# WeChatCV/WeDetect

Measured on AMD Instinct MI355X. Metric: images/s at 640x640 (WeDetect-Base image tower + 80-class similarity + top-k/NMS), higher is better.
Workload: dtype f32-equivalent: fp32 operands carried as fp16 hi+lo pairs, 3 fp16-MFMA passes per product, fp32 accumulate (fp16x3); similarity GEMM, dwconv, LN, post-process native f32

## Files before the change

### wedetect_amd/csrc/split_gemm.hip

```cpp
#include <stdlib.h>
#include "split_gemm_impl.h"

namespace {

__global__ void split_weights_kernel(const float* __restrict__ w, int n, int k, int k16, float scale,
                                     unsigned short* __restrict__ out, int n_out) {
  const long long idx = (long long)blockIdx.x * blockDim.x + threadIdx.x;
  if (idx >= (long long)n_out * k16) return;
  const int row = (int)(idx / k16), kk = (int)(idx % k16);
  const float x = (kk < k && row < n) ? w[(size_t)row * k + kk] * scale : 0.0f;
  const _Float16 hi = (_Float16)x;
  const _Float16 lo = (_Float16)(x - (float)hi);
  unsigned short* o = out + (size_t)row * 2 * k16 + (kk >> 3) * 16 + (kk & 7);
  o[0] = __builtin_bit_cast(unsigned short, hi);
  o[8] = __builtin_bit_cast(unsigned short, lo);
}

template <int ACT, bool SPECIAL>
__global__ void __launch_bounds__(256) splitk_reduce_kernel(const WdConvGemm p, const float* __restrict__ ws, int splits,
                                                            float unscale, int vec_c, int vec_res, int vec_bias) {
  const long long idx = (long long)blockIdx.x * blockDim.x + threadIdx.x;
  const int nq = p.n >> 2;
  if (idx >= (long long)p.m * nq) return;
  const int m = (int)(idx / nq), n = (int)(idx - (long long)m * nq) * 4;
  const size_t plane = (size_t)p.m * p.n;
  f32x4 v = *reinterpret_cast<const f32x4*>(ws + (size_t)m * p.n + n);
  for (int s = 1; s < splits; ++s) v += *reinterpret_cast<const f32x4*>(ws + s * plane + (size_t)m * p.n + n);
  const EpiVec ev{vec_c, vec_res, vec_bias, unscale};
  epi_quad<ACT, SPECIAL>(p, epi_row<SPECIAL>(p, m), ev, m, n, v);
}

template <bool SPECIAL>
int launch_reduce(const WdConvGemm& p, const float* ws, int splits, float unscale, hipStream_t st) {
  const long long total = (long long)p.m * (p.n >> 2);
  const dim3 grid((unsigned)((total + 255) / 256)), block(256);
  const int vec_c = (p.ldc % 4 == 0) && wd_aligned16(p.c) && (p.out_mode == WD_OUT_ROWS || (p.n % 16 == 0));
  const int vec_res = p.res ? ((p.ldres % 4 == 0) && wd_aligned16(p.res)) : 0;
  const int vec_bias = p.bias ? wd_aligned16(p.bias) : 0;
  switch (p.act) {
    case WD_ACT_RELU: hipLaunchKernelGGL((splitk_reduce_kernel<WD_ACT_RELU, SPECIAL>), grid, block, 0, st, p, ws, splits, unscale, vec_c, vec_res, vec_bias); break;
    case WD_ACT_SILU: hipLaunchKernelGGL((splitk_reduce_kernel<WD_ACT_SILU, SPECIAL>), grid, block, 0, st, p, ws, splits, unscale, vec_c, vec_res, vec_bias); break;
    case WD_ACT_GELU: hipLaunchKernelGGL((splitk_reduce_kernel<WD_ACT_GELU, SPECIAL>), grid, block, 0, st, p, ws, splits, unscale, vec_c, vec_res, vec_bias); break;
    default: hipLaunchKernelGGL((splitk_reduce_kernel<WD_ACT_NONE, SPECIAL>), grid, block, 0, st, p, ws, splits, unscale, vec_c, vec_res, vec_bias); break;
  }
  return wd_launch_status();
}

}

extern "C" int64_t wd_split_weights_bytes(int32_t n, int32_t k) {
  if (n <= 0 || k <= 0) return 0;
  return (int64_t)((n + 7) & ~7) * ((k + 15) / 16 * 16) * 4;
}

static int split_weights_launch(const float* w, int32_t n, int32_t k, float scale, void* out, void* stream, int n_out) {
  if (!w || !out || n <= 0 || k <= 0 || !(scale > 0.0f) || !wd_aligned16(out)) return WD_ERR_BAD_ARG;
  const int k16 = (k + 15) / 16 * 16;
  const long long total = (long long)n_out * k16;
  hipLaunchKernelGGL(split_weights_kernel, dim3((unsigned)((total + 255) / 256)), dim3(256), 0,
                     static_cast<hipStream_t>(stream), w, n, k, k16, scale, static_cast<unsigned short*>(out), n_out);
  return wd_launch_status();
}

extern "C" int wd_split_weights(const float* w, int32_t n, int32_t k, float scale, void* out, void* stream) {
  return split_weights_launch(w, n, k, scale, out, stream, n);
}

extern "C" int wd_split_weights_padded(const float* w, int32_t n, int32_t k, float scale, void* out, void* stream) {
  return split_weights_launch(w, n, k, scale, out, stream, (n + 7) & ~7);
}

static int pick_split_cfg(const WdConvGemm& p) {
  const int m = p.m, n = p.n;
  const long long pad128 = (long long)((n + 127) / 128) * 128, pad64 = (long long)((n + 63) / 64) * 64;
  if (pad64 < pad128) return m >= 65536 ? 52 : 53;
  const bool plain = p.kh == 1 && p.kw == 1 && p.stride == 1 && p.pad == 0;
  if (plain && p.k >= 1024) return 55;
  const long long tiles = (long long)((m + 127) / 128) * ((n + 127) / 128);
  return tiles < 1024 ? 50 : 51;
}

long long wd_p8_workspace_floats();
bool wd_p8_persist_ok(int m, int n);
bool wd_conv_pp_ok(const WdConvGemm& p, int flags);
int wd_launch_conv_pp(const WdConvGemm& p, const void* w, float unscale, int flags, hipStream_t st, int ksplits, float* ws,
                      long long ws_floats, int variant, const float* unscale_dev = nullptr);
bool wd_conv3_ok(const WdConvGemm& p, int flags);
const char* wd_conv3_config_name(int m, int n);
int wd_launch_conv3(const WdConvGemm& p, const void* w, float unscale, int flags, hipStream_t st, int variant, int ksplits, float* ws,
                    long long ws_floats);

extern "C" int64_t wd_p8_workspace_bytes(void) { return 4 * wd_p8_workspace_floats(); }

static int pick_presplit_cfg(int m, int n, int k, bool park) {
  if (k % 32 == 0 && k >= 256 && m % 8 == 0 && n % 256 == 0) {
    const long long tiles = (long long)((m + 255) / 256) * (n / 256);
    static const int mink = [] { const char* e = getenv("WD_P8_PERSIST_MINK"); return e ? atoi(e) : 1024; }();
    if (park && k >= mink && wd_p8_persist_ok(m, n)) return 65;
    if (tiles >= 128) return 64;
  }
  if (k % 16 == 0 && n % 256 == 0 && m % 16 == 0 && m >= 131072) return 66;
  return m >= 131072 ? 63 : 60;
}

extern "C" const char* wd_conv_gemm_split_config(int32_t m, int32_t n, int32_t k, int32_t is_conv) {
  if (is_conv == 4) {
    const bool narrow = (n % 128) != 0 && ((n + 63) / 64) * 64 < ((n + 127) / 128) * 128;
    return narrow ? "fp16x3 256x64x16/8w/dma" : "fp16x3 256x128x16/8w/dma";
  }
  if (is_conv == 5) return wd_conv3_config_name(m, n);
  if ((is_conv == 2 || is_conv == 3) && k % 16 == 0) {
    switch (pick_presplit_cfg(m, n, k, is_conv == 3)) {
      case 65: return "fp16x3 256x256x32/8w/p8s";
      case 64: return "fp16x3 256x256x32/8w/p8";
      case 66: return "fp16x3 128x256x16/4w/p4";
      case 63: return "fp16x3 256x128x16/8w/pingpong";
      default: return "fp16x3 128x128x16/4w/glds";
    }
  }
  WdConvGemm q{};
  q.m = m; q.n = n; q.k = k; q.kh = q.kw = q.stride = 1;
  if (is_conv) q.kh = q.kw = 3;
  switch (pick_split_cfg(q)) {
    case 50: return "fp16x3 128x128x32/4w";
    case 51: return "fp16x3 128x128x16/4w";
    case 52: return "fp16x3 256x64x16/4w";
    case 55: return "fp16x3 128x128x32/4w/pf2";
    default: return "fp16x3 128x64x16/2w";
  }
}

static int pick_ksplits(const WdConvGemm& p, int cfg, int flags, long long ws_floats) {
  if (ws_floats <= 0 || (flags & WD_SPLIT_C) || (p.n & 3) || cfg == 55 || cfg == 63 || cfg >= 64) return 1;
  const int bm = 128, bn = (cfg == 52 || cfg == 53) ? 64 : 128, bk = (cfg == 50) ? 32 : 16;
  const long long tiles = (long long)((p.m + (cfg == 52 ? 255 : bm - 1)) / (cfg == 52 ? 256 : bm)) * ((p.n + bn - 1) / bn);
  const int nk = (p.k + bk - 1) / bk;
  if (tiles >= 128 || nk < 16) return 1;
  int s = (int)(512 / tiles);
  if (s > nk / 8) s = nk / 8;
  if (s > 16) s = 16;
  while (s > 1 && (long long)s * p.m * p.n > ws_floats) --s;
  return s < 2 ? 1 : s;
}

static int conv_gemm_split_impl(const WdConvGemm* pp, const void* w_split, float w_unscale, int32_t flags, int32_t cfg,
                                float* ws, int64_t ws_bytes, int32_t force_splits, hipStream_t st) {
  if (!pp) return WD_ERR_BAD_ARG;
  const WdConvGemm& p = *pp;
  const int rc = check_split_args(p, w_split, w_unscale);
  if (rc != WD_OK) return rc;
  if (flags & ~(WD_SPLIT_A | WD_SPLIT_C)) return WD_ERR_BAD_ARG;
  if (ws && !wd_aligned16(ws)) return WD_ERR_BAD_ARG;
  if (p.c2 && !(flags & WD_SPLIT_C)) return WD_ERR_BAD_ARG;
  const bool production = cfg < 0;
  if (cfg < 0) cfg = pick_split_cfg(p);
  const bool plain = p.kh == 1 && p.kw == 1 && p.stride == 1 && p.pad == 0;
  const bool special = p.out_mode != WD_OUT_ROWS || p.c_batch_stride > 0 || p.seg_rows > 0 || p.sigmoid ||
                       p.out_scale != 1.0f || p.out_bias != 0.0f;
  if (p.ln_stats || p.ln_u) {
    if (!p.ln_stats || !p.ln_u || flags != (WD_SPLIT_A | WD_SPLIT_C) || !plain || special || p.res || p.c2 || force_splits > 1 ||
        !wd_aligned16(p.ln_u) || (reinterpret_cast<uintptr_t>(p.ln_stats) & 7u))
      return WD_ERR_BAD_ARG;
    if (cfg == 70 || cfg == 73 || cfg == 74 || (cfg >= 75 && cfg <= 79) || (cfg >= 700 && cfg < 716)) return WD_ERR_UNSUPPORTED;
  }
  if (flags & WD_SPLIT_A) {
    const bool covered = plain && !special && !p.c2 && !((flags & WD_SPLIT_C) && p.res);
    const bool forced = cfg == 70 || cfg == 73 || cfg == 74 || (cfg >= 700 && cfg < 716);
    static const bool conv3_on = [] { const char* e = getenv("WEDETECT_CONV3"); return !(e && e[0] == '0'); }();
    if ((cfg >= 75 && cfg <= 79) || (production && conv3_on && !(force_splits == 0 && ws != nullptr))) {
      if (wd_conv3_ok(p, flags) && wd_conv_pp_ok(p, flags))
        return wd_launch_conv3(p, w_split, w_unscale, flags, st, cfg == 76 ? 2 : cfg == 77 ? 7 : cfg == 78 ? 8 : cfg == 79 ? 9 : 0, force_splits > 1 ? force_splits : 1, ws, ws ? ws_bytes / 4 : 0);
      if (cfg >= 75 && cfg <= 79) return WD_ERR_UNSUPPORTED;
    }
    if (forced || (production && !covered)) {
      if (!wd_conv_pp_ok(p, flags)) return forced || !covered ? WD_ERR_UNSUPPORTED : WD_ERR_BAD_ARG;
      const long long wsf = ws ? ws_bytes / 4 : 0;
      int splits = force_splits > 0 ? force_splits : 1;
      if (force_splits == 0 && wsf > 0 && !forced) {
        const long long tiles = (long long)((p.m + 255) / 256) * ((p.n + 127) / 128);
        const int nk = p.k / 16;
        if (tiles < 128 && nk >= 32) {
          int s2 = (int)(256 / tiles);
          if (s2 > nk / 16) s2 = nk / 16;
          if (s2 > 8) s2 = 8;
          while (s2 > 1 && (long long)s2 * p.m * p.n > wsf) --s2;
          if (s2 > 1) splits = s2;
        }
      }
      return wd_launch_conv_pp(p, w_split, w_unscale, flags, st, splits, ws, wsf,
                               cfg == 73 ? 3 : cfg == 74 ? 4 : cfg >= 700 ? cfg - 600 : 0);
    }
  }
  if (flags == WD_SPLIT_C) {
    if (!plain || special || p.res || p.c2 || p.n % 8 || p.ldc % 8 || (p.bias && !wd_aligned16(p.bias)) || !wd_aligned16(p.c))
      return WD_ERR_UNSUPPORTED;
    constexpr int VC = SVAR_XCD | SVAR_PIN | SVAR_LDSEPI | SVAR_CSPLIT;
    const long long tiles = (long long)((p.m + 127) / 128) * ((p.n + 127) / 128);
    return tiles < 1024 ? launch_split<2, 2, 2, 2, 32, VC, 1>(p, w_split, w_unscale, st)
                        : launch_split<2, 2, 2, 2, 16, VC, 1>(p, w_split, w_unscale, st);
  }
  if (flags != 0) {
    if (production && plain && !special && p.k % 16 == 0)
      cfg = pick_presplit_cfg(p.m, p.n, p.k, ws != nullptr && force_splits == 0 && ws_bytes / 4 >= wd_p8_workspace_floats() &&
                                                 p.lda % 8 == 0 && !(flags & ~(WD_SPLIT_A | WD_SPLIT_C)));
    if (cfg != 50 && cfg != 51 && cfg != 55 && cfg != 60 && cfg != 63 && cfg != 64 && cfg != 65 && cfg != 66 && !(cfg >= 640 && cfg < 768)) cfg = 51;
    if ((flags & WD_SPLIT_C) && cfg == 55) cfg = 50;
  }
  const long long ws_floats = ws ? ws_bytes / 4 : 0;
  int splits = force_splits > 0 ? force_splits : pick_ksplits(p, cfg, flags, ws_floats);
  {
    const int bk = (cfg == 50) ? 32 : 16, nk = (p.k + bk - 1) / bk;
    if (splits > nk) splits = nk;
  }
  if (splits > 1) {
    if ((flags & WD_SPLIT_C) || (p.n & 3) || cfg == 55 || cfg == 63 || cfg >= 64) return WD_ERR_UNSUPPORTED;
    if ((long long)splits * p.m * p.n > ws_floats) return WD_ERR_WORKSPACE;
  }
  int lrc;
  if (flags != 0) {
    lrc = wd_launch_presplit(p, w_split, w_unscale, cfg, flags, st, splits, ws, ws_floats);
  } else {
    switch (cfg) {
      case 41: lrc = launch_split<2, 2, 2, 4, 16, SVAR_XCD | SVAR_PIN | SVAR_LDSEPI>(p, w_split, w_unscale, st, splits, ws); break;
      case 50: lrc = launch_split<2, 2, 2, 2, 32, SVAR_XCD | SVAR_PIN | SVAR_LDSEPI>(p, w_split, w_unscale, st, splits, ws); break;
      case 51: lrc = launch_split<2, 2, 2, 2, 16, SVAR_XCD | SVAR_PIN | SVAR_LDSEPI>(p, w_split, w_unscale, st, splits, ws); break;
      case 52: lrc = launch_split<2, 2, 4, 1, 16, SVAR_XCD | SVAR_PIN | SVAR_LDSEPI>(p, w_split, w_unscale, st, splits, ws); break;
      case 53: lrc = launch_split<2, 2, 2, 1, 16, SVAR_XCD | SVAR_PIN | SVAR_LDSEPI>(p, w_split, w_unscale, st, splits, ws); break;
      case 55: lrc = launch_split<2, 2, 2, 2, 32, SVAR_XCD | SVAR_PF2 | SVAR_LDSEPI>(p, w_split, w_unscale, st); break;
      default: return WD_ERR_UNSUPPORTED;
    }
  }
  if (lrc != WD_OK || splits <= 1) return lrc;
  return special ? launch_reduce<true>(p, ws, splits, w_unscale, st) : launch_reduce<false>(p, ws, splits, w_unscale, st);
}

extern "C" int wd_conv_gemm_split(const WdConvGemm* pp, const void* w_split, float w_unscale, int32_t flags,
                                  int32_t cfg, void* stream) {
  return conv_gemm_split_impl(pp, w_split, w_unscale, flags, cfg, nullptr, 0, 0, static_cast<hipStream_t>(stream));
}

extern "C" int wd_conv_gemm_split_ws(const WdConvGemm* pp, const void* w_split, float w_unscale, int32_t flags,
                                     int32_t cfg, void* workspace, int64_t workspace_bytes, int32_t splits, void* stream) {
  if (splits < 0 || workspace_bytes < 0) return WD_ERR_BAD_ARG;
  return conv_gemm_split_impl(pp, w_split, w_unscale, flags, cfg, static_cast<float*>(workspace), workspace_bytes, splits,
                              static_cast<hipStream_t>(stream));
}

extern "C" int wd_fold_similarity(const WdConvGemm* pp, const void* w_split, float w_unscale, const float* w_unscale_dev,
                                  void* stream) {
  if (!pp || !w_unscale_dev) return WD_ERR_BAD_ARG;
  const WdConvGemm& p = *pp;
  const int rc = check_split_args(p, w_split, w_unscale);
  if (rc != WD_OK) return rc;
  if (p.kh != 1 || p.kw != 1 || p.stride != 1 || p.pad != 0 || p.c_batch_stride <= 0 || p.res || p.c2 || p.ln_stats || p.ln_u ||
      p.seg_rows > 0 || p.act != WD_ACT_NONE)
// ... 5 lines not shown
```

### wedetect_amd/csrc/split_gemm_conv3.hip

```cpp
#include <stdlib.h>
#include "split_epi_oct.h"

namespace {

constexpr int C3_BM = 256, C3_AG = 17;
constexpr int C3_AROWS = C3_AG * 16, C3_ROWB = 64;

__device__ __forceinline__ void c3_dma16(unsigned lds_addr, const unsigned char* src) {
  asm volatile("s_mov_b32 m0, %0\n\tglobal_load_lds_dwordx4 %1, off" ::"s"(lds_addr), "v"(src) : "memory", "m0");
}

template <int TN, int NBUF_ = 3>
struct C3 {
  static constexpr int WROWS = 64 * TN;
  static constexpr int WG = WROWS / 16;
  static constexpr int NG = C3_AG + 3 * WG;
  static constexpr int NJ = (NG + 7) / 8;
  static constexpr int A_BYTES = C3_AROWS * C3_ROWB;
  static constexpr int STAGE = A_BYTES + 3 * WROWS * C3_ROWB + 1024;
  static constexpr int NBUF = NBUF_;
  static constexpr int LDS = NBUF * STAGE;
  static_assert(LDS <= 160 * 1024, "LDS");
  static_assert(NJ == 6 || NJ == 4, "the counted waits of the K loop");
  static_assert(LDS >= 8 * 32 * EPI_LDT * 4, "operand LDS must hold one epilogue patch per wave");
};

#define C3_BARRIER()                          \
  do {                                        \
    __builtin_amdgcn_sched_barrier(0);        \
    asm volatile("" ::: "memory");            \
    __builtin_amdgcn_s_barrier();             \
    asm volatile("" ::: "memory");            \
    __builtin_amdgcn_sched_barrier(0);        \
  } while (0)

template <int TN, bool CSPLIT, int NB = 3, bool STAG = false>
__global__ void __launch_bounds__(512, NB == 2 ? 4 : 2)
split_conv3_kernel(const WdConvGemm p, const unsigned char* __restrict__ wsp, const float* __restrict__ zero, int k16,
                   float unscale, int nbn, int ksplits, float* __restrict__ ws) {
  using T = C3<TN, NB>;
  constexpr int TM = 2, BM = C3_BM, BN = 64 * TN, ROWB = C3_ROWB, NJ = T::NJ, NBUF = T::NBUF, DIST = NBUF - 1;
  extern __shared__ __attribute__((aligned(16))) unsigned char smem_raw[];
  const int t = threadIdx.x, lane = t & 63, wave = t >> 6;
  const int group = wave >> 2, wm = (wave >> 1) & 1, wn = wave & 1;
  int tile = blockIdx.x;
  {
    const int nwg = gridDim.x, xcd = tile & 7, idx = tile >> 3;
    const int q = nwg >> 3, r = nwg & 7;
    tile = (xcd < r ? xcd * (q + 1) : r * (q + 1) + (xcd - r) * q) + idx;
  }
  const int ntiles = gridDim.x / ksplits;
  const int ks = tile / ntiles;
  tile -= ks * ntiles;
  const int bn = tile % nbn, bm = tile / nbn;
  const int m0 = bm * BM, n0 = bn * BN;
  const int nci = p.cin >> 4, nk_all = 3 * nci;
  const int per_split = (nk_all + ksplits - 1) / ksplits;
  const int s_begin = ks * per_split;
  const int nk = (s_begin + per_split < nk_all ? s_begin + per_split : nk_all) - s_begin;

  const unsigned char* base[NJ];
  unsigned vmask[NJ];
  int kind[NJ], tapoff[NJ];
  unsigned ldst[NJ];
  const unsigned char* zp = reinterpret_cast<const unsigned char*>(zero);
#pragma unroll
  for (int j = 0; j < NJ; ++j) {
    const int g = wave + 8 * j;
    const int rl = lane >> 2;
    if (g < C3_AG) {
      const int row = g * 16 + rl;
      const int logical = (lane & 3) ^ ((row >> 2) & 3);
      const int memchunk = ((logical & 1) << 1) | ((logical >> 1) & 1);
      const long long mc = (long long)m0 - 1 + row;
      const bool ok = row < BM + 2 && mc >= 0 && mc < p.m;
      const long long mm = ok ? mc : 0;
      const int ho = (int)((mm / p.wout) % p.hout);
      base[j] = reinterpret_cast<const unsigned char*>(p.a) + mm * p.lda * 4 + memchunk * 16;
      unsigned mk = 0;
#pragma unroll
      for (int kh = 0; kh < 3; ++kh) mk |= ((unsigned)(ho + kh - 1) < (unsigned)p.hin) ? (1u << kh) : 0u;
      vmask[j] = ok ? mk : 0u;
      kind[j] = 0; tapoff[j] = 0;
      ldst[j] = (unsigned)(g * 1024);
    } else if (g < T::NG) {
      const int gw = g - C3_AG, tap = gw / T::WG, r16 = gw - tap * T::WG;
      const int row = r16 * 16 + rl;
      const int logical = (lane & 3) ^ ((row >> 2) & 3);
      const int memchunk = ((logical & 1) << 1) | ((logical >> 1) & 1);
      const int n = n0 + row;
      const bool ok = n < p.n;
      base[j] = wsp + (size_t)(ok ? n : 0) * k16 * 4 + memchunk * 16;
      vmask[j] = ok ? 7u : 0u;
      kind[j] = 1; tapoff[j] = tap * p.cin * 4;
      ldst[j] = (unsigned)(T::A_BYTES + (tap * T::WROWS + r16 * 16) * ROWB);
    } else {
      base[j] = zp; vmask[j] = 0u; kind[j] = 2; tapoff[j] = 0;
      ldst[j] = (unsigned)(T::STAGE - 1024);
    }
  }
  const unsigned lds0 = (unsigned)(size_t)(__attribute__((address_space(3))) unsigned char*)smem_raw;
  int i_kh = s_begin / nci, i_ci = (s_begin - (s_begin / nci) * nci) * 16;
  auto issue_part = [&](int buf, auto j0_c, auto j1_c, auto last_c) {
    constexpr int J0 = decltype(j0_c)::value, J1 = decltype(j1_c)::value;
    const unsigned lbase = lds0 + buf * T::STAGE;
    const int a_off = ((i_kh - 1) * p.wout * p.lda + i_ci) * 4;
// ... 129 lines not shown
    for (int s = 0; s < nk; ++s) {
      const unsigned char* sp = smem_raw + bcur * T::STAGE;
      const bool more = s + 2 < nk;
      rd(sp, 0);
      C3_SBARRIER();
      mm();
      C3_SBARRIER();
      rd(sp, 1);
      if (more) issue_part(bfill, IC0{}, ICH{}, std::false_type{});
      C3_SBARRIER();
      mm();
      C3_SBARRIER();
      rd(sp, 2);
      if (more) {
        issue_part(bfill, ICH{}, ICN{}, std::true_type{});
        if constexpr (NJ == 6) asm volatile("s_waitcnt vmcnt(6)" ::: "memory");
        else asm volatile("s_waitcnt vmcnt(4)" ::: "memory");
      } else {
        asm volatile("s_waitcnt vmcnt(0)" ::: "memory");
      }
      C3_SBARRIER();
      mm();
      C3_SBARRIER();
      bcur = bcur == 2 ? 0 : bcur + 1;
      bfill = bfill == 2 ? 0 : bfill + 1;
    }
    if (group == 0) C3_SBARRIER();
    C3_SBARRIER();
  } else {
#pragma unroll
  for (int d = 0; d < DIST; ++d)
    if (d < nk) issue(d);
  asm volatile("s_waitcnt vmcnt(0)" ::: "memory");
  __syncthreads();
  int bcur = 0, bfill = DIST % NBUF;
  for (int s = 0; s < nk; ++s) {
    const unsigned char* sp = smem_raw + bcur * T::STAGE;
    if (s + DIST < nk) issue(bfill);
    __builtin_amdgcn_sched_barrier(0);
    tap(sp, 0);
    tap(sp, 1);
    tap(sp, 2);
    __builtin_amdgcn_sched_barrier(0);
    if (DIST == 2 && s + 2 <= nk - 1) {
      if constexpr (NJ == 6) asm volatile("s_waitcnt vmcnt(6)" ::: "memory");
      else asm volatile("s_waitcnt vmcnt(4)" ::: "memory");
    } else {
      asm volatile("s_waitcnt vmcnt(0)" ::: "memory");
    }
    __builtin_amdgcn_sched_barrier(0);
    __syncthreads();
    __builtin_amdgcn_sched_barrier(0);
    bcur = bcur == NBUF - 1 ? 0 : bcur + 1;
    bfill = bfill == NBUF - 1 ? 0 : bfill + 1;
  }
  __syncthreads();
  }

  const int mw = m0 + group * 128 + wm * 64, nw = n0 + wn * 32 * TN;
  float* patch = reinterpret_cast<float*>(smem_raw) + wave * 32 * EPI_LDT;
  if (ksplits > 1) {
    WdConvGemm pr = p;
    pr.bias = nullptr; pr.res = nullptr; pr.c2 = nullptr; pr.range_flag = nullptr;
    pr.c = ws + (size_t)ks * p.m * p.n; pr.ldc = p.n;
    pr.out_mode = WD_OUT_ROWS; pr.c_batch_stride = 0; pr.seg_rows = 0; pr.sigmoid = 0; pr.out_scale = 1.0f; pr.out_bias = 0.0f;
    pr.act = WD_ACT_NONE;
    EpiOctOperands<TM, TN, false> ops;
    ops.load(pr, mw, nw, lane);
    EpiOctWalk<0, TM, TN, WD_ACT_NONE, false, false, false>::run(pr, 1.0f, mw, nw, lane, acc, patch, ops);
    return;
  }
  epi_oct_all<TM, TN, CSPLIT, TN == 1>(p, unscale, mw, nw, lane, acc, patch);
#ifdef C3_TRACE
  if constexpr (STAG) {
    asm volatile("s_waitcnt vmcnt(0)" ::: "memory");
    if (tile == 0 && ks == 0 && (wave & 3) == 0 && ws && lane == 0) {
      unsigned long long* trc = reinterpret_cast<unsigned long long*>(ws) + (wave >> 2) * 4096;
      trc[4095] = __builtin_readcyclecounter();
    }
  }
#endif
}

template <int TN, bool CSPLIT>
__global__ void __launch_bounds__(768, 1)
split_conv3w_kernel(const WdConvGemm p, const unsigned char* __restrict__ wsp, const float* __restrict__ zero, int k16,
                    float unscale, int nbn, int ksplits, float* __restrict__ ws) {
  using T = C3<TN, 3>;
  constexpr int TM = 2, BM = C3_BM, BN = 64 * TN, ROWB = C3_ROWB;
  constexpr int NJP = (T::NG + 3) / 4;
  static_assert(4 * NJP * 1024 <= T::STAGE + 3 * 1024, "spare slots");
  static_assert(NJP == 11 || NJP == 8, "the counted waits of the producer loop");
  extern __shared__ __attribute__((aligned(16))) unsigned char smem_raw[];
  const int t = threadIdx.x, lane = t & 63;
  const int wave = __builtin_amdgcn_readfirstlane(t >> 6);
  int tile = blockIdx.x;
  {
    const int nwg = gridDim.x, xcd = tile & 7, idx = tile >> 3;
    const int q = nwg >> 3, r = nwg & 7;
    tile = (xcd < r ? xcd * (q + 1) : r * (q + 1) + (xcd - r) * q) + idx;
  }
  const int ntiles = gridDim.x / ksplits;
  const int ks = tile / ntiles;
  tile -= ks * ntiles;
  const int bn = tile % nbn, bm = tile / nbn;
  const int m0 = bm * BM, n0 = bn * BN;
  const int nci = p.cin >> 4, nk_all = 3 * nci;
  const int per_split = (nk_all + ksplits - 1) / ksplits;
  const int s_begin = ks * per_split;
  const int nk = (s_begin + per_split < nk_all ? s_begin + per_split : nk_all) - s_begin;
  const unsigned lds0 = (unsigned)(size_t)(__attribute__((address_space(3))) unsigned char*)smem_raw;
#ifdef C3_TRACE
  unsigned long long* trc = (tile == 0 && ks == 0 && (wave & 3) == 0 && ws) ? reinterpret_cast<unsigned long long*>(ws) + (wave >> 2) * 4096 : nullptr;
  int trc_i = 0;
  C3_STAMP();
#endif

  if (wave >= 8) {
    const int pw = wave - 8;
    const unsigned char* zp = reinterpret_cast<const unsigned char*>(zero);
    const unsigned char* base[NJP];
    unsigned vmask[NJP];
#pragma unroll
    for (int j = 0; j < NJP; ++j) {
      const int g = pw + 4 * j;
      const int rl = lane >> 2;
      if (g < C3_AG) {
        const int row = g * 16 + rl;
        const int logical = (lane & 3) ^ ((row >> 2) & 3);
        const int memchunk = ((logical & 1) << 1) | ((logical >> 1) & 1);
        const int mc = m0 - 1 + row;
        const bool ok = row < BM + 2 && mc >= 0 && mc < p.m;
        const unsigned mm = ok ? (unsigned)mc : 0u;
        const int ho = (int)((mm / (unsigned)p.wout) % (unsigned)p.hout);
        base[j] = reinterpret_cast<const unsigned char*>(p.a) + (size_t)mm * p.lda * 4 + memchunk * 16;
        unsigned mk = 0;
#pragma unroll
        for (int kh = 0; kh < 3; ++kh) mk |= ((unsigned)(ho + kh - 1) < (unsigned)p.hin) ? (1u << kh) : 0u;
        vmask[j] = ok ? mk : 0u;
      } else if (g < T::NG) {
        const int gw = g - C3_AG, tap = gw / T::WG, r16 = gw - tap * T::WG;
        const int row = r16 * 16 + rl;
        const int logical = (lane & 3) ^ ((row >> 2) & 3);
        const int memchunk = ((logical & 1) << 1) | ((logical >> 1) & 1);
        const int n = n0 + row;
        const bool ok = n < p.n;
        base[j] = wsp + (size_t)(ok ? n : 0) * k16 * 4 + memchunk * 16 + (size_t)tap * p.cin * 4;
        vmask[j] = ok ? 7u : 0u;
      } else {
        base[j] = zp; vmask[j] = 0u;
      }
    }
    int i_kh = s_begin / nci, i_ci = (s_begin - (s_begin / nci) * nci) * 16;
    auto issue = [&](int buf) {
      const unsigned lbase = lds0 + buf * T::STAGE;
      const int a_off = ((i_kh - 1) * p.wout * p.lda + i_ci) * 4;
      const int w_off = (i_kh * 3 * p.cin + i_ci) * 4;
#pragma unroll
      for (int j = 0; j < NJP; ++j) {
        const int g = pw + 4 * j;
        const bool is_a = g < C3_AG;
        const unsigned ldst = is_a ? (unsigned)(g * 1024)
                                   : (g < T::NG ? (unsigned)(T::A_BYTES + (((g - C3_AG) / T::WG) * T::WROWS + ((g - C3_AG) % T::WG) * 16) * ROWB)
                                                : (unsigned)(T::STAGE - 1024));
        const unsigned bit = is_a ? (vmask[j] >> i_kh) & 1u : vmask[j] & 1u;
        c3_dma16(__builtin_amdgcn_readfirstlane(lbase + ldst), bit ? base[j] + (is_a ? a_off : w_off) : zp);
      }
      i_ci += 16;
      if (i_ci == p.cin) { i_ci = 0; ++i_kh; }
    };
    if (0 < nk) issue(0);
    if (1 < nk) issue(1);
    int bfill = 2;
    for (int k = 0; k < nk; ++k) {
      if (k + 1 < nk) {
        if constexpr (NJP == 11) asm volatile("s_waitcnt vmcnt(11)" ::: "memory");
        else asm volatile("s_waitcnt vmcnt(8)" ::: "memory");
      } else {
        asm volatile("s_waitcnt vmcnt(0)" ::: "memory");
      }
      C3_SBARRIER();
      if (k + 2 < nk) issue(bfill);
      bfill = bfill == 2 ? 0 : bfill + 1;
    }
    C3_SBARRIER();
    return;
  }

  const int group = wave >> 2, wm = (wave >> 1) & 1, wn = wave & 1;
  f32x16 acc[TM][TN];
#pragma unroll
  for (int i = 0; i < TM; ++i)
#pragma unroll
    for (int j = 0; j < TN; ++j)
#pragma unroll
      for (int r = 0; r < 16; ++r) acc[i][j][r] = 0.0f;
  unsigned aoff_h[3][TM], aoff_l[3][TM], boff_h[TN], boff_l[TN];
  const int hsel = lane >> 5;
#pragma unroll
  for (int i = 0; i < TM; ++i) {
    const int q = group * 128 + wm * 64 + i * 32 + (lane & 31);
#pragma unroll
    for (int kw = 0; kw < 3; ++kw) {
      const int row = q + kw, f = (row >> 2) & 3;
      aoff_h[kw][i] = lds0 + row * ROWB + ((hsel ^ f) << 4);
      aoff_l[kw][i] = lds0 + row * ROWB + (((2 + hsel) ^ f) << 4);
    }
    const unsigned wo = (unsigned)(m0 + q) % (unsigned)p.wout;
    constexpr unsigned ZROW = (C3_BM + 8) * ROWB;
    if (wo == 0u) { aoff_h[0][i] = lds0 + ZROW; aoff_l[0][i] = lds0 + ZROW + 32; }
    if (wo == (unsigned)p.wout - 1u) { aoff_h[2][i] = lds0 + ZROW; aoff_l[2][i] = lds0 + ZROW + 32; }
  }
#pragma unroll
  for (int j = 0; j < TN; ++j) {
    const int row = wn * 32 * TN + j * 32 + (lane & 31), f = (row >> 2) & 3;
    boff_h[j] = lds0 + T::A_BYTES + row * ROWB + ((hsel ^ f) << 4);
    boff_l[j] = lds0 + T::A_BYTES + row * ROWB + (((2 + hsel) ^ f) << 4);
  }
  h8 xh[2][TM] = {}, xl[2][TM] = {}, wh[2][TN] = {}, wl[2][TN] = {};
  using K0 = std::integral_constant<int, 0>;
  using K1 = std::integral_constant<int, 1>;
  using K2 = std::integral_constant<int, 2>;
  auto tap = [&](unsigned nb, auto kwn_c, auto cur_c) {
    constexpr int KWN = decltype(kwn_c)::value, C = decltype(cur_c)::value, N = 1 - C;
    constexpr int NR = 2 * TM + 2 * TN;
    unsigned ra[NR];
#pragma unroll
    for (int i = 0; i < TM; ++i) { ra[2 * i] = nb + aoff_h[KWN][i]; ra[2 * i + 1] = nb + aoff_l[KWN][i]; }
#pragma unroll
    for (int jj = 0; jj < TN; ++jj) {
      ra[2 * TM + 2 * jj] = nb + KWN * (T::WROWS * ROWB) + boff_h[jj];
      ra[2 * TM + 2 * jj + 1] = nb + KWN * (T::WROWS * ROWB) + boff_l[jj];
    }
    asm volatile("s_waitcnt lgkmcnt(0)" ::: "memory");
    __builtin_amdgcn_s_setprio(1);
#pragma unroll
    for (int m = 0; m < 3 * TM * TN; ++m) {
      const int pass = m / (TM * TN), i = (m % (TM * TN)) / TN, jj = m % TN;
      if (pass == 0) asm volatile("v_mfma_f32_32x32x16_f16 %0, %1, %2, %0" : "+v"(acc[i][jj]) : "v"(wl[C][jj]), "v"(xh[C][i]));
      else if (pass == 1) asm volatile("v_mfma_f32_32x32x16_f16 %0, %1, %2, %0" : "+v"(acc[i][jj]) : "v"(wh[C][jj]), "v"(xl[C][i]));
      else asm volatile("v_mfma_f32_32x32x16_f16 %0, %1, %2, %0" : "+v"(acc[i][jj]) : "v"(wh[C][jj]), "v"(xh[C][i]));
      if (m < NR) {
        const int r = m;
        if (r < 2 * TM) {
          if (r & 1) asm volatile("ds_read_b128 %0, %1" : "=v"(xl[N][r >> 1]) : "v"(ra[r]) : "memory");
          else asm volatile("ds_read_b128 %0, %1" : "=v"(xh[N][r >> 1]) : "v"(ra[r]) : "memory");
        } else {
          if (r & 1) asm volatile("ds_read_b128 %0, %1" : "=v"(wl[N][(r - 2 * TM) >> 1]) : "v"(ra[r]) : "memory");
          else asm volatile("ds_read_b128 %0, %1" : "=v"(wh[N][(r - 2 * TM) >> 1]) : "v"(ra[r]) : "memory");
        }
      }
    }
    __builtin_amdgcn_s_setprio(0);
  };
  auto stage = [&](unsigned sb, unsigned sbn, auto p0_c) {
    constexpr int P0 = decltype(p0_c)::value;
    using S0 = std::integral_constant<int, P0>;
    using S1 = std::integral_constant<int, 1 - P0>;
    tap(sb, K1{}, S0{});
    tap(sb, K2{}, S1{});
    asm volatile("s_waitcnt lgkmcnt(0)" ::: "memory");
    C3_SBARRIER();
    tap(sbn, K0{}, S0{});
  };
  C3_SBARRIER();
#pragma unroll
  for (int i = 0; i < TM; ++i) {
    asm volatile("ds_read_b128 %0, %1" : "=v"(xh[0][i]) : "v"(aoff_h[0][i]) : "memory");
    asm volatile("ds_read_b128 %0, %1" : "=v"(xl[0][i]) : "v"(aoff_l[0][i]) : "memory");
  }
#pragma unroll
  for (int jj = 0; jj < TN; ++jj) {
    asm volatile("ds_read_b128 %0, %1" : "=v"(wh[0][jj]) : "v"(boff_h[jj]) : "memory");
    asm volatile("ds_read_b128 %0, %1" : "=v"(wl[0][jj]) : "v"(boff_l[jj]) : "memory");
  }
  int bcur = 0;
  for (int s = 0; s < nk; s += 2) {
    const int b1 = bcur == 2 ? 0 : bcur + 1, b2 = b1 == 2 ? 0 : b1 + 1;
    stage((unsigned)(bcur * T::STAGE), (unsigned)(b1 * T::STAGE), K0{});
    if (s + 1 < nk) stage((unsigned)(b1 * T::STAGE), (unsigned)(b2 * T::STAGE), K1{});
    bcur = b2;
  }
  asm volatile("s_waitcnt lgkmcnt(0)" ::: "memory");

  const int mw = m0 + group * 128 + wm * 64, nw = n0 + wn * 32 * TN;
  float* patch = reinterpret_cast<float*>(smem_raw) + wave * 32 * EPI_LDT;
  if (ksplits > 1) {
    WdConvGemm pr = p;
    pr.bias = nullptr; pr.res = nullptr; pr.c2 = nullptr; pr.range_flag = nullptr;
    pr.c = ws + (size_t)ks * p.m * p.n; pr.ldc = p.n;
    pr.out_mode = WD_OUT_ROWS; pr.c_batch_stride = 0; pr.seg_rows = 0; pr.sigmoid = 0; pr.out_scale = 1.0f; pr.out_bias = 0.0f;
    pr.act = WD_ACT_NONE;
    EpiOctOperands<TM, TN, false> ops;
    ops.load(pr, mw, nw, lane);
    EpiOctWalk<0, TM, TN, WD_ACT_NONE, false, false, false>::run(pr, 1.0f, mw, nw, lane, acc, patch, ops);
    return;
  }
  epi_oct_all<TM, TN, CSPLIT, TN == 1>(p, unscale, mw, nw, lane, acc, patch);
#ifdef C3_TRACE
  asm volatile("s_waitcnt vmcnt(0)" ::: "memory");
  if (trc && lane == 0) trc[4095] = __builtin_readcyclecounter();
#endif
}

template <int TN, bool CSPLIT>
int launch_conv3w(const WdConvGemm& p, const void* wsp, float unscale, hipStream_t st, int ksplits = 1, float* ws = nullptr) {
  using T = C3<TN, 3>;
  constexpr int BN = 64 * TN;
  const int nbm = (p.m + C3_BM - 1) / C3_BM, nbn = (p.n + BN - 1) / BN;
  const long long nblk = (long long)nbm * nbn * ksplits;
  if (nblk <= 0 || nblk > 0x7fffffffLL || (long long)p.m + 2 * C3_BM >= 0x7fffffffLL) return WD_ERR_BAD_ARG;
  const int k16 = (p.k + 15) / 16 * 16;
  const float* zero = wd_zero_block();
  if (!zero) return WD_ERR_LAUNCH;
  auto k = split_conv3w_kernel<TN, CSPLIT>;
  static WdAttrOnce attr;
  if (wd_set_max_lds(attr, reinterpret_cast<const void*>(k), T::LDS) != WD_OK) return WD_ERR_LAUNCH;
  WD_LAUNCH_GEMM(k, dim3((unsigned)nblk), dim3(768), T::LDS, st, p, static_cast<const unsigned char*>(wsp), zero, k16, unscale, nbn,
                 ksplits, ws);
  return wd_launch_status();
}

template <int TN, bool CSPLIT, int NB = 3, bool STAG = false>
int launch_conv3(const WdConvGemm& p, const void* wsp, float unscale, hipStream_t st, int ksplits = 1, float* ws = nullptr) {
  using T = C3<TN, NB>;
  constexpr int BN = 64 * TN;
  const int nbm = (p.m + C3_BM - 1) / C3_BM, nbn = (p.n + BN - 1) / BN;
  const long long nblk = (long long)nbm * nbn * ksplits;
  if (nblk <= 0 || nblk > 0x7fffffffLL) return WD_ERR_BAD_ARG;
  const int k16 = (p.k + 15) / 16 * 16;
  const float* zero = wd_zero_block();
  if (!zero) return WD_ERR_LAUNCH;
  auto k = split_conv3_kernel<TN, CSPLIT, NB, STAG>;
  static WdAttrOnce attr;
  if (wd_set_max_lds(attr, reinterpret_cast<const void*>(k), T::LDS) != WD_OK) return WD_ERR_LAUNCH;
  WD_LAUNCH_GEMM(k, dim3((unsigned)nblk), dim3(512), T::LDS, st, p, static_cast<const unsigned char*>(wsp), zero, k16, unscale, nbn,
                 ksplits, ws);
  return wd_launch_status();
}

}

bool wd_conv3_ok(const WdConvGemm& p, int flags) {
  if (!(flags & WD_SPLIT_A)) return false;
  if (p.kh != 3 || p.kw != 3 || p.stride != 1 || p.pad != 1 || p.hout != p.hin || p.wout != p.win) return false;
  if (p.cin % 16 || p.k != 9 * p.cin || p.lda % 8 || p.n % 8 || p.wout < 2) return false;
  if ((unsigned long long)p.m * p.lda * 4 >= (1ull << 40)) return false;
  return true;
}

int wd_launch_oct_reduce(const WdConvGemm& p, const float* ws, int splits, float unscale, bool csplit, hipStream_t st);

static bool conv3_stag_default() {
  static const bool on = [] { const char* e = getenv("WEDETECT_CONV3_STAG"); return !(e && e[0] == '0'); }();
  return on;
}

static bool conv3_ws_default() {
  static const bool on = [] { const char* e = getenv("WEDETECT_CONV3_WS"); return !(e && e[0] == '0'); }();
  return on;
}

int wd_launch_conv3(const WdConvGemm& p, const void* w, float unscale, int flags, hipStream_t st, int variant, int ksplits,
                    float* ws, long long ws_floats) {
  if (!wd_conv3_ok(p, flags)) return WD_ERR_UNSUPPORTED;
  const bool csplit = (flags & WD_SPLIT_C) != 0;
  const bool w12 = variant == 9 || (variant == 0 && conv3_ws_default());
  const bool stag = variant == 7 || (variant != 8 && conv3_stag_default());
  const bool narrow = (p.n % 128) != 0 && ((p.n + 63) / 64) * 64 < ((p.n + 127) / 128) * 128;
  if (ksplits < 1) ksplits = 1;
#ifdef C3_TRACE
  float* tws = ws;
#else
  float* tws = nullptr;
#endif
  if (ksplits > 1) {
    if (!ws || (long long)ksplits * p.m * p.n > ws_floats) return WD_ERR_WORKSPACE;
    if (ksplits > 3 * (p.cin >> 4)) ksplits = 3 * (p.cin >> 4);
    int rc;
    if (w12) {
      if (narrow) rc = csplit ? launch_conv3w<1, true>(p, w, unscale, st, ksplits, ws) : launch_conv3w<1, false>(p, w, unscale, st, ksplits, ws);
      else rc = csplit ? launch_conv3w<2, true>(p, w, unscale, st, ksplits, ws) : launch_conv3w<2, false>(p, w, unscale, st, ksplits, ws);
    } else if (stag) {
      if (narrow) rc = csplit ? launch_conv3<1, true, 3, true>(p, w, unscale, st, ksplits, ws) : launch_conv3<1, false, 3, true>(p, w, unscale, st, ksplits, ws);
      else rc = csplit ? launch_conv3<2, true, 3, true>(p, w, unscale, st, ksplits, ws) : launch_conv3<2, false, 3, true>(p, w, unscale, st, ksplits, ws);
    } else {
      if (narrow) rc = csplit ? launch_conv3<1, true>(p, w, unscale, st, ksplits, ws) : launch_conv3<1, false>(p, w, unscale, st, ksplits, ws);
      else rc = csplit ? launch_conv3<2, true>(p, w, unscale, st, ksplits, ws) : launch_conv3<2, false>(p, w, unscale, st, ksplits, ws);
    }
    if (rc != WD_OK) return rc;
    return wd_launch_oct_reduce(p, ws, ksplits, unscale, csplit, st);
  }
  if (narrow) {
    const long long tiles = (long long)((p.m + C3_BM - 1) / C3_BM) * ((p.n + 63) / 64);
    const bool ring2 = variant == 2 || ((variant == 0 || variant == 8) && tiles > 256);
    if (variant == 9) return csplit ? launch_conv3w<1, true>(p, w, unscale, st, 1, tws) : launch_conv3w<1, false>(p, w, unscale, st, 1, tws);
    if (ring2) return csplit ? launch_conv3<1, true, 2>(p, w, unscale, st) : launch_conv3<1, false, 2>(p, w, unscale, st);
    if (w12) return csplit ? launch_conv3w<1, true>(p, w, unscale, st, 1, tws) : launch_conv3w<1, false>(p, w, unscale, st, 1, tws);
    if (stag) return csplit ? launch_conv3<1, true, 3, true>(p, w, unscale, st) : launch_conv3<1, false, 3, true>(p, w, unscale, st);
    return csplit ? launch_conv3<1, true>(p, w, unscale, st) : launch_conv3<1, false>(p, w, unscale, st);
  }
  if (w12) return csplit ? launch_conv3w<2, true>(p, w, unscale, st, 1, tws) : launch_conv3w<2, false>(p, w, unscale, st, 1, tws);
  if (stag) return csplit ? launch_conv3<2, true, 3, true>(p, w, unscale, st, 1, tws) : launch_conv3<2, false, 3, true>(p, w, unscale, st, 1, tws);
  return csplit ? launch_conv3<2, true>(p, w, unscale, st) : launch_conv3<2, false>(p, w, unscale, st);
}

const char* wd_conv3_config_name(int m, int n) {
  const bool narrow = (n % 128) != 0 && ((n + 63) / 64) * 64 < ((n + 127) / 128) * 128;
  const bool w12 = conv3_ws_default();
  if (narrow) {
    const long long tiles = (long long)((m + C3_BM - 1) / C3_BM) * ((n + 63) / 64);
    if (tiles > 256) return "fp16x3 256x64x16/8w/dma3/ring2";
    return w12 ? "fp16x3 256x64x16/12w/dma3" : "fp16x3 256x64x16/8w/dma3";
  }
  return w12 ? "fp16x3 256x128x16/12w/dma3" : "fp16x3 256x128x16/8w/dma3";
}
```

Baseline: 1011.

## Add warp-specialized DMA implicit-GEMM path for stride-2 3x3 convolutions

Adds a stride-2 variant of the warp-specialized conv3 kernel: producer waves DMA per-tap A rows (with padding masks) and weight rows directly into LDS in two-step stages, and consumer waves run the fp16x3 MFMA loop over them. It is enabled by default for production stride-2 3x3 pad-1 convs that previously fell to the generic split-GEMM/im2col-style path. The aim is to cut global traffic and launch overhead for downsampling convs. In exchange it adds another specialized path with a tight counted-wait pipeline and one barrier per step.

```diff
diff --git a/wedetect_amd/csrc/split_gemm.hip b/wedetect_amd/csrc/split_gemm.hip
--- a/wedetect_amd/csrc/split_gemm.hip
+++ b/wedetect_amd/csrc/split_gemm.hip
@@ -89,6 +89,10 @@
 const char* wd_conv3_config_name(int m, int n);
 int wd_launch_conv3(const WdConvGemm& p, const void* w, float unscale, int flags, hipStream_t st, int variant, int ksplits, float* ws,
                     long long ws_floats);
+
+bool wd_conv3s2_ok(const WdConvGemm& p, int flags);
+bool wd_conv3s2_default();
+int wd_launch_conv3s2(const WdConvGemm& p, const void* w, float unscale, int flags, hipStream_t st);
 
 extern "C" int64_t wd_p8_workspace_bytes(void) { return 4 * wd_p8_workspace_floats(); }
 
@@ -161,7 +165,7 @@
     if (!p.ln_stats || !p.ln_u || flags != (WD_SPLIT_A | WD_SPLIT_C) || !plain || special || p.res || p.c2 || force_splits > 1 ||
         !wd_aligned16(p.ln_u) || (reinterpret_cast<uintptr_t>(p.ln_stats) & 7u))
       return WD_ERR_BAD_ARG;
-    if (cfg == 70 || cfg == 73 || cfg == 74 || (cfg >= 75 && cfg <= 79) || (cfg >= 700 && cfg < 716)) return WD_ERR_UNSUPPORTED;
+    if (cfg == 70 || cfg == 73 || cfg == 74 || (cfg >= 75 && cfg <= 80) || (cfg >= 700 && cfg < 716)) return WD_ERR_UNSUPPORTED;
   }
   if (flags & WD_SPLIT_A) {
     const bool covered = plain && !special && !p.c2 && !((flags & WD_SPLIT_C) && p.res);
@@ -171,6 +175,11 @@
       if (wd_conv3_ok(p, flags) && wd_conv_pp_ok(p, flags))
         return wd_launch_conv3(p, w_split, w_unscale, flags, st, cfg == 76 ? 2 : cfg == 77 ? 7 : cfg == 78 ? 8 : cfg == 79 ? 9 : 0, force_splits > 1 ? force_splits : 1, ws, ws ? ws_bytes / 4 : 0);
       if (cfg >= 75 && cfg <= 79) return WD_ERR_UNSUPPORTED;
+    }
+    if (cfg == 80 || (production && force_splits <= 1 && !(force_splits == 0 && ws != nullptr) && wd_conv3s2_default())) {
+      if (wd_conv3s2_ok(p, flags) && wd_conv_pp_ok(p, flags) && (cfg == 80 ? force_splits <= 1 : true))
+        return wd_launch_conv3s2(p, w_split, w_unscale, flags, st);
+      if (cfg == 80) return WD_ERR_UNSUPPORTED;
     }
     if (forced || (production && !covered)) {
       if (!wd_conv_pp_ok(p, flags)) return forced || !covered ? WD_ERR_UNSUPPORTED : WD_ERR_BAD_ARG;
diff --git a/wedetect_amd/csrc/split_gemm_conv3.hip b/wedetect_amd/csrc/split_gemm_conv3.hip
--- a/wedetect_amd/csrc/split_gemm_conv3.hip
+++ b/wedetect_amd/csrc/split_gemm_conv3.hip
@@ -22,6 +22,21 @@
   static constexpr int LDS = NBUF * STAGE;
   static_assert(LDS <= 160 * 1024, "LDS");
   static_assert(NJ == 6 || NJ == 4, "the counted waits of the K loop");
+  static_assert(LDS >= 8 * 32 * EPI_LDT * 4, "operand LDS must hold one epilogue patch per wave");
+};
+
+template <int TN>
+struct C3S2 {
+  static constexpr int WROWS = 64 * TN;
+  static constexpr int WG = WROWS / 16;
+  static constexpr int SG = 16 + WG;
+  static constexpr int A_BYTES = 16 * 1024;
+  static constexpr int SUB = SG * 1024;
+  static constexpr int NG = 2 * SG;
+  static constexpr int STAGE = NG * 1024;
+  static constexpr int LDS = 3 * STAGE;
+  static_assert(SG % 4 == 0, "slot j and slot j + NJP / 2 of a producer cover the same rows of the stage's two steps");
+  static_assert(LDS <= 160 * 1024, "LDS");
   static_assert(LDS >= 8 * 32 * EPI_LDT * 4, "operand LDS must hold one epilogue patch per wave");
 };
 
@@ -317,15 +332,17 @@
 #endif
 }
 
-template <int TN, bool CSPLIT>
+template <int TN, bool CSPLIT, int STRIDE = 1>
 __global__ void __launch_bounds__(768, 1)
 split_conv3w_kernel(const WdConvGemm p, const unsigned char* __restrict__ wsp, const float* __restrict__ zero, int k16,
                     float unscale, int nbn, int ksplits, float* __restrict__ ws) {
-  using T = C3<TN, 3>;
+  static_assert(STRIDE == 1 || STRIDE == 2, "stride");
+  constexpr bool S2 = STRIDE == 2;
+  using T = std::conditional_t<S2, C3S2<TN>, C3<TN, 3>>;
   constexpr int TM = 2, BM = C3_BM, BN = 64 * TN, ROWB = C3_ROWB;
   constexpr int NJP = (T::NG + 3) / 4;
   static_assert(4 * NJP * 1024 <= T::STAGE + 3 * 1024, "spare slots");
-  static_assert(NJP == 11 || NJP == 8, "the counted waits of the producer loop");
+  static_assert(S2 ? (NJP == 12 || NJP == 10) : (NJP == 11 || NJP == 8), "the counted waits of the producer loop");
   extern __shared__ __attribute__((aligned(16))) unsigned char smem_raw[];
   const int t = threadIdx.x, lane = t & 63;
   const int wave = __builtin_amdgcn_readfirstlane(t >> 6);
@@ -340,7 +357,8 @@
   tile -= ks * ntiles;
   const int bn = tile % nbn, bm = tile / nbn;
   const int m0 = bm * BM, n0 = bn * BN;
-  const int nci = p.cin >> 4, nk_all = 3 * nci;
+  const int nci = p.cin >> 4;
+  const int nk_all = S2 ? ((p.k >> 4) + 1) >> 1 : 3 * nci;
   const int per_split = (nk_all + ksplits - 1) / ksplits;
   const int s_begin = ks * per_split;
   const int nk = (s_begin + per_split < nk_all ? s_begin + per_split : nk_all) - s_begin;
@@ -354,6 +372,81 @@
   if (wave >= 8) {
     const int pw = wave - 8;
     const unsigned char* zp = reinterpret_cast<const unsigned char*>(zero);
+    if constexpr (S2) {
+      constexpr int NH = NJP / 2;
+      const unsigned char* base[NH];
+      unsigned vmask[NH];
+#pragma unroll
+      for (int j = 0; j < NH; ++j) {
+        const int g = pw + 4 * j;
+        const int row = (g < 16 ? g : g - 16) * 16 + (lane >> 2);
+        const int logical = (lane & 3) ^ ((row >> 2) & 3);
+        const int memchunk = ((logical & 1) << 1) | ((logical >> 1) & 1);
+        if (g < 16) {
+          const int m = m0 + row;
+          const bool ok = m < p.m;
+          const int mm = ok ? m : 0;
+          const int wo = mm % p.wout, q = mm / p.wout;
+          const int ho = q % p.hout, b = q / p.hout;
+          const int hi0 = ho * 2 - 1, wi0 = wo * 2 - 1;
+          const long long pix = ((long long)b * p.hin + hi0) * p.win + wi0;
+          base[j] = reinterpret_cast<const unsigned char*>(p.a) + pix * p.lda * 4 + memchunk * 16;
+          unsigned mk = 0, bit = 1u;
+#pragma unroll
+          for (int kh = 0; kh < 3; ++kh) {
+            const bool hok = (unsigned)(hi0 + kh) < (unsigned)p.hin;
+#pragma unroll
+            for (int kw = 0; kw < 3; ++kw, bit <<= 1) mk |= (hok && (unsigned)(wi0 + kw) < (unsigned)p.win) ? bit : 0u;
+          }
+          vmask[j] = ok ? mk : 0u;
+        } else {
+          const int n = n0 + row;
+          const bool ok = n < p.n;
+          base[j] = wsp + (size_t)(ok ? n : 0) * k16 * 4 + memchunk * 16;
+          vmask[j] = ok ? 0x1FFu : 0u;
+        }
+      }
+      const int nsteps = p.k >> 4;
+      int i_step = 0, i_tap = 0, i_kh = 0, i_kw = 0, i_ci = 0;
+      auto issue = [&](int buf) {
+        const unsigned lbase = lds0 + buf * T::STAGE;
+#pragma unroll
+        for (int u = 0; u < 2; ++u) {
+          const bool live = i_step < nsteps;
+          const int a_off = ((i_kh * p.win + i_kw) * p.lda + i_ci) * 4;
+          const int w_off = i_step * ROWB;
+#pragma unroll
+          for (int j = 0; j < NH; ++j) {
+            const int g = pw + 4 * j;
+            const bool is_a = g < 16;
+            const unsigned bit = live ? (is_a ? (vmask[j] >> i_tap) & 1u : vmask[j] & 1u) : 0u;
+            c3_dma16(__builtin_amdgcn_readfirstlane(lbase + (unsigned)(u * T::SUB + g * 1024)), bit ? base[j] + (is_a ? a_off : w_off) : zp);
+          }
+          ++i_step;
+          i_ci += 16;
+          if (i_ci == p.cin) {
+            i_ci = 0; ++i_tap;
+            if (++i_kw == 3) { i_kw = 0; ++i_kh; }
+          }
+        }
+      };
+      if (0 < nk) issue(0);
+      if (1 < nk) issue(1);
+      int bfill = 2;
+      for (int k = 0; k < nk; ++k) {
+        if (k + 1 < nk) {
+          if constexpr (NJP == 12) asm volatile("s_waitcnt vmcnt(12)" ::: "memory");
+          else asm volatile("s_waitcnt vmcnt(10)" ::: "memory");
+        } else {
+          asm volatile("s_waitcnt vmcnt(0)" ::: "memory");
+        }
+        C3_SBARRIER();
+        if (k + 2 < nk) issue(bfill);
+        bfill = bfill == 2 ? 0 : bfill + 1;
+      }
+      C3_SBARRIER();
+      return;
+    } else {
     const unsigned char* base[NJP];
     unsigned vmask[NJP];
 #pragma unroll
@@ -420,6 +513,7 @@
     }
     C3_SBARRIER();
     return;
+    }
   }
 
   const int group = wave >> 2, wm = (wave >> 1) & 1, wn = wave & 1;
@@ -430,6 +524,7 @@
     for (int j = 0; j < TN; ++j)
 #pragma unroll
       for (int r = 0; r < 16; ++r) acc[i][j][r] = 0.0f;
+  constexpr unsigned WSTEP = S2 ? (unsigned)T::NG / 2 * 1024u : (unsigned)(T::WROWS * ROWB);
   unsigned aoff_h[3][TM], aoff_l[3][TM], boff_h[TN], boff_l[TN];
   const int hsel = lane >> 5;
 #pragma unroll
@@ -437,14 +532,17 @@
     const int q = group * 128 + wm * 64 + i * 32 + (lane & 31);
 #pragma unroll
     for (int kw = 0; kw < 3; ++kw) {
-      const int row = q + kw, f = (row >> 2) & 3;
-      aoff_h[kw][i] = lds0 + row * ROWB + ((hsel ^ f) << 4);
-      aoff_l[kw][i] = lds0 + row * ROWB + (((2 + hsel) ^ f) << 4);
-    }
-    const unsigned wo = (unsigned)(m0 + q) % (unsigned)p.wout;
-    constexpr unsigned ZROW = (C3_BM + 8) * ROWB;
-    if (wo == 0u) { aoff_h[0][i] = lds0 + ZROW; aoff_l[0][i] = lds0 + ZROW + 32; }
-    if (wo == (unsigned)p.wout - 1u) { aoff_h[2][i] = lds0 + ZROW; aoff_l[2][i] = lds0 + ZROW + 32; }
+      const int row = S2 ? q : q + kw, f = (row >> 2) & 3;
+      const unsigned so = S2 ? (kw & 1) * WSTEP : 0u;
+      aoff_h[kw][i] = lds0 + so + row * ROWB + ((hsel ^ f) << 4);
+      aoff_l[kw][i] = lds0 + so + row * ROWB + (((2 + hsel) ^ f) << 4);
+    }
+    if constexpr (!S2) {
+      const unsigned wo = (unsigned)(m0 + q) % (unsigned)p.wout;
+      constexpr unsigned ZROW = (C3_BM + 8) * ROWB;
+      if (wo == 0u) { aoff_h[0][i] = lds0 + ZROW; aoff_l[0][i] = lds0 + ZROW + 32; }
+      if (wo == (unsigned)p.wout - 1u) { aoff_h[2][i] = lds0 + ZROW; aoff_l[2][i] = lds0 + ZROW + 32; }
+    }
   }
 #pragma unroll
   for (int j = 0; j < TN; ++j) {
@@ -464,8 +562,8 @@
     for (int i = 0; i < TM; ++i) { ra[2 * i] = nb + aoff_h[KWN][i]; ra[2 * i + 1] = nb + aoff_l[KWN][i]; }
 #pragma unroll
     for (int jj = 0; jj < TN; ++jj) {
-      ra[2 * TM + 2 * jj] = nb + KWN * (T::WROWS * ROWB) + boff_h[jj];
-      ra[2 * TM + 2 * jj + 1] = nb + KWN * (T::WROWS * ROWB) + boff_l[jj];
+      ra[2 * TM + 2 * jj] = nb + KWN * WSTEP + boff_h[jj];
+      ra[2 * TM + 2 * jj + 1] = nb + KWN * WSTEP + boff_l[jj];
     }
     asm volatile("s_waitcnt lgkmcnt(0)" ::: "memory");
     __builtin_amdgcn_s_setprio(1);
@@ -510,11 +608,22 @@
     asm volatile("ds_read_b128 %0, %1" : "=v"(wl[0][jj]) : "v"(boff_l[jj]) : "memory");
   }
   int bcur = 0;
+  if constexpr (S2) {
+    for (int s = 0; s < nk; ++s) {
+      const int b1 = bcur == 2 ? 0 : bcur + 1;
+      tap((unsigned)(bcur * T::STAGE), K1{}, K0{});
+      asm volatile("s_waitcnt lgkmcnt(0)" ::: "memory");
+      C3_SBARRIER();
+      tap((unsigned)(b1 * T::STAGE), K0{}, K1{});
+      bcur = b1;
+    }
+  } else {
   for (int s = 0; s < nk; s += 2) {
     const int b1 = bcur == 2 ? 0 : bcur + 1, b2 = b1 == 2 ? 0 : b1 + 1;
     stage((unsigned)(bcur * T::STAGE), (unsigned)(b1 * T::STAGE), K0{});
     if (s + 1 < nk) stage((unsigned)(b1 * T::STAGE), (unsigned)(b2 * T::STAGE), K1{});
     bcur = b2;
+  }
   }
   asm volatile("s_waitcnt lgkmcnt(0)" ::: "memory");
 
@@ -538,9 +647,9 @@
 #endif
 }
 
-template <int TN, bool CSPLIT>
+template <int TN, bool CSPLIT, int STRIDE = 1>
 int launch_conv3w(const WdConvGemm& p, const void* wsp, float unscale, hipStream_t st, int ksplits = 1, float* ws = nullptr) {
-  using T = C3<TN, 3>;
+  using T = std::conditional_t<STRIDE == 2, C3S2<TN>, C3<TN, 3>>;
   constexpr int BN = 64 * TN;
   const int nbm = (p.m + C3_BM - 1) / C3_BM, nbn = (p.n + BN - 1) / BN;
   const long long nblk = (long long)nbm * nbn * ksplits;
@@ -548,7 +657,7 @@
   const int k16 = (p.k + 15) / 16 * 16;
   const float* zero = wd_zero_block();
   if (!zero) return WD_ERR_LAUNCH;
-  auto k = split_conv3w_kernel<TN, CSPLIT>;
+  auto k = split_conv3w_kernel<TN, CSPLIT, STRIDE>;
   static WdAttrOnce attr;
   if (wd_set_max_lds(attr, reinterpret_cast<const void*>(k), T::LDS) != WD_OK) return WD_ERR_LAUNCH;
   WD_LAUNCH_GEMM(k, dim3((unsigned)nblk), dim3(768), T::LDS, st, p, static_cast<const unsigned char*>(wsp), zero, k16, unscale, nbn,
@@ -640,6 +749,28 @@
   return csplit ? launch_conv3<2, true>(p, w, unscale, st) : launch_conv3<2, false>(p, w, unscale, st);
 }
 
+bool wd_conv3s2_ok(const WdConvGemm& p, int flags) {
+  if (!(flags & WD_SPLIT_A)) return false;
+  if (p.kh != 3 || p.kw != 3 || p.stride != 2 || p.pad != 1 || p.hin < 1 || p.win < 1) return false;
+  if (p.hout != (p.hin - 1) / 2 + 1 || p.wout != (p.win - 1) / 2 + 1) return false;
+  if (p.cin % 16 || p.k != 9 * p.cin || p.lda % 8 || p.lda < p.cin || p.n % 8) return false;
+  if ((unsigned long long)p.m * 4 * p.lda * 4 >= (1ull << 40)) return false;
+  return true;
+}
+
+bool wd_conv3s2_default() {
+  const char* e = getenv("WEDETECT_CONV3_S2");
+  return !(e && e[0] == '0');
+}
+
+int wd_launch_conv3s2(const WdConvGemm& p, const void* w, float unscale, int flags, hipStream_t st) {
+  if (!wd_conv3s2_ok(p, flags)) return WD_ERR_UNSUPPORTED;
+  const bool csplit = (flags & WD_SPLIT_C) != 0;
+  const bool narrow = (p.n % 128) != 0 && ((p.n + 63) / 64) * 64 < ((p.n + 127) / 128) * 128;
+  if (narrow) return csplit ? launch_conv3w<1, true, 2>(p, w, unscale, st) : launch_conv3w<1, false, 2>(p, w, unscale, st);
+  return csplit ? launch_conv3w<2, true, 2>(p, w, unscale, st) : launch_conv3w<2, false, 2>(p, w, unscale, st);
+}
+
 const char* wd_conv3_config_name(int m, int n) {
   const bool narrow = (n % 128) != 0 && ((n + 63) / 64) * 64 < ((n + 127) / 128) * 128;
   const bool w12 = conv3_ws_default();
```

After: 1013 (median of 6 runs). No clear change (+0.2%).
